# jhhung/kISS

Hardware: AMD Instinct MI355X
Metric: bases/sec suffix_sort (chm13v2.0-size synthetic, k=256) (higher is better)
Workload: dtype u8; 1 GPU; suffix_sort genome-like synthetic n=3117292070 k=256 (stand-in for chm13v2.0.fa, BASELINE.json configs[1]); PARALLEL_SORTING; text resident in HBM, SA left in HBM; n=3117292070, k=256, seed=2, parallelism=single GPU, lms=905939973, lms_rounds=9, tied_after_round0_item_rounds=184319413, big_segment_item_rounds=72866550, workspace_bytes=80357006484, induce_passes=47

## Files before the change

### kiss_amd/csrc/api.hip

```cpp
#include "kiss_internal.hpp"
#include <cstdlib>
#include <chrono>
#include <mutex>
#include <cstring>
#include <new>

KTimer::KTimer(kiss_hip_ctx *c, int cls, uint64_t items) : ctx(c), idx(-1)
{
    if (!((ctx->profile_mask >> cls) & 1ull)) return;
    if (ctx->ev_used == ctx->ev_pool.size()) {
        kiss_hip_ctx::Ev e;
        if (hipEventCreate(&e.a) != hipSuccess || hipEventCreate(&e.b) != hipSuccess) return;
        e.cls = 0;
        ctx->ev_pool.push_back(e);
    }
    idx = (int)ctx->ev_used++;
    ctx->ev_pool[idx].cls = cls;
    ctx->stats.launches_kernel[cls]++;
    ctx->stats.items_kernel[cls] += items;
    (void)hipEventRecord(ctx->ev_pool[idx].a, ctx->stream);
}
KTimer::~KTimer()
{
    if (idx >= 0) (void)hipEventRecord(ctx->ev_pool[idx].b, ctx->stream);
// ... 35 lines not shown
    o.pair_keys = env_on("KISS_HIP_PAIR_KEYS");
    o.no_fc0_onepass = env_on("KISS_HIP_NO_FC0_ONEPASS");
    o.no_pair_records = env_on("KISS_HIP_NO_PAIR_RECORDS");
    o.no_small_fused = env_on("KISS_HIP_NO_SMALL_FUSED");
    o.no_class_bytes = env_on("KISS_HIP_NO_CLASS_BYTES");
    o.no_pivot_ctx = env_on("KISS_HIP_NO_PIVOT_CTX");
    o.no_taint = env_on("KISS_HIP_NO_TAINT");
    o.isa_direct = env_on("KISS_HIP_ISA_DIRECT");
    o.no_onesweep = env_on("KISS_HIP_NO_ONESWEEP");
    o.rx_one_tile = env_on("KISS_HIP_RX_ONE_TILE");
    o.merge_lms = env_on("KISS_HIP_MERGE_LMS");
    o.no_small_alphabet = env_on("KISS_HIP_NO_SMALL_ALPHABET");
    o.induce_one_pass = env_on("KISS_HIP_INDUCE_ONE_PASS");
    o.verify = env_on("KISS_HIP_VERIFY");
    o.no_prefault = env_on("KISS_HIP_NO_PREFAULT");
    o.doubling_h0 = (uint32_t)env_u64("KISS_HIP_DOUBLING_H0", 0);
    o.tcap0 = env_u64("KISS_HIP_TCAP0", 0);
    o.pivot_slots = (int)env_u64("KISS_HIP_PIVOT_SLOTS", 3);
    o.small_seg = (uint32_t)env_u64("KISS_HIP_SMALL_SEG", 0);
    o.near_merge_min = (uint32_t)env_u64("KISS_HIP_NEAR_MERGE_MIN", 4096);
    o.induce_small_max = (uint32_t)env_u64("KISS_HIP_INDUCE_SMALL_MAX", 0);
    o.collapse_cap = (uint32_t)env_u64("KISS_HIP_COLLAPSE_CAP", 0);
    o.collapse_n = env_u64("KISS_HIP_COLLAPSE_N", 0);
    o.fm_heavy = (uint32_t)env_u64("KISS_HIP_FM_HEAVY", 0);
    o.fm_light = (uint32_t)env_u64("KISS_HIP_FM_LIGHT", 0);
    o.fm_mm_wave = env_on("KISS_HIP_FM_MM_WAVE");
    o.fm_mm_budget = env_u64("KISS_HIP_FM_MM_BUDGET", 0);
    o.fm8_group = env_on("KISS_HIP_FM8_GROUP");
    o.isa_direct_max = env_u64("KISS_HIP_ISA_DIRECT_MAX", 0);
    o.lx_sync_points = (unsigned)env_u64("KISS_HIP_LX_SYNC_POINTS", 0);
    o.tie_trace = (unsigned)env_u64("KISS_HIP_TIE_TRACE", 0);
    o.poison = (uint32_t)env_u64("KISS_HIP_POISON", 0);
    if (const char *e = getenv("KISS_HIP_DUMP_PIVOT")) snprintf(o.dump_pivot, sizeof o.dump_pivot, "%s", e);
    ctx->opts = o;
}
static std::mutex &kiss_launch_mutex()
{
    static std::mutex m;
    return m;
}
static bool kiss_lock_launches()
{
    static const bool on = getenv("KISS_HIP_LOCK_LAUNCHES") != nullptr;
    return on;
}
bool kiss_sync_launches()
// ... 98 lines not shown
    ctx->t_cap = 0;
    ctx->flags_cap = 0;
}

void free_lms_side(kiss_hip_ctx *ctx)
{
    free_tied(ctx);
    void **ptrs[] = {(void **)&ctx->lms_pos, (void **)&ctx->keyA, (void **)&ctx->keyB, (void **)&ctx->posA,
                     (void **)&ctx->posB, (void **)&ctx->lms_sorted_far, (void **)&ctx->lms_ctx_far,
                     (void **)&ctx->lmsP, (void **)&ctx->lmsC, (void **)&ctx->tile_hist, (void **)&ctx->scan_tmp,
                     (void **)&ctx->rx_desc, (void **)&ctx->rx_ghist, (void **)&ctx->fc_desc};
    for (void **p : ptrs)
        if (*p) {
            (void)hipFree(*p);
            *p = nullptr;
        }
    ctx->ws_bytes -= ctx->lms_bytes;
    ctx->lms_bytes = 0;
}

void free_all(kiss_hip_ctx *ctx)
{
    free_lms_side(ctx);
    void *ptrs[] = {ctx->pk, ctx->tile_gp, ctx->tile_cnt, ctx->cl_part, ctx->d_counts, ctx->CTX, ctx->CLS, ctx->ind_counts, ctx->ind_desc,
                    ctx->d_small, ctx->near_idx, ctx->near_fin, ctx->near_pos, ctx->near_tmp, ctx->near_tmp2, ctx->pairs1, ctx->pairs2, ctx->rx_ctl, ctx->refine_heads, ctx->ga_codes};
    for (void *p : ptrs)
        if (p) (void)hipFree(p);
    for (void *p : ctx->fm_pool)
        if (p) (void)hipFree(p);
    for (hipEvent_t e : ctx->fm_mm_ev)
        if (e) (void)hipEventDestroy(e);
#ifdef KISS_HIP_HOOKS
    if (ctx->tie_dbg) (void)hipFree(ctx->tie_dbg);
#endif
    if (ctx->io_S) (void)hipFree(ctx->io_S);
    if (ctx->io_SA) (void)hipFree(ctx->io_SA);
    kiss_xfer_free(ctx);
    if (ctx->h_pinned) (void)hipHostFree(ctx->h_pinned);
    if (ctx->h_pub) (void)hipHostFree(ctx->h_pub);
    for (auto &e : ctx->ev_pool) {
        (void)hipEventDestroy(e.a);
        (void)hipEventDestroy(e.b);
    }
    if (ctx->own_stream) (void)hipStreamDestroy(ctx->own_stream);
}

int sort_dev_unlocked(kiss_hip_ctx *ctx, const uint8_t *d_S, uint64_t n, uint32_t k, int algo, uint32_t *d_SA, void *stream);
int sort_dev(kiss_hip_ctx *ctx, const uint8_t *d_S, uint64_t n, uint32_t k, int algo, uint32_t *d_SA, void *stream)
{
    if (!ctx) return KISS_HIP_E_INVALID;
    kiss_opts_refresh(ctx);
#ifdef KISS_NO_DEVICE_LOCK
    return sort_dev_unlocked(ctx, d_S, n, k, algo, d_SA, stream);
#endif
    if (ctx->opts.no_serialize) return sort_dev_unlocked(ctx, d_S, n, k, algo, d_SA, stream);
    std::lock_guard<std::mutex> lock(kiss_device_mutex(ctx->device));
// ... 129 lines not shown

int kiss_need_ctx_words(kiss_hip_ctx *ctx)
{
    if (ctx->CTX && ctx->CLS) return KISS_HIP_OK;
    if (!ctx->CTX) KTRY(dmalloc(ctx, &ctx->CTX, ctx->max_n + 2));
    if (!ctx->CLS) KTRY(dmalloc(ctx, &ctx->CLS, ctx->max_n + 2 + 64));
    return KISS_HIP_OK;
}

int kiss_lms_reserve(kiss_hip_ctx *ctx, uint64_t m_cap, uint64_t t_cap_wanted)
{
    const bool dbg = ctx->opts.debug;
    const auto t_begin = std::chrono::steady_clock::now();
    free_lms_side(ctx);
    if (dbg)
        fprintf(stderr, "[kiss_hip] lms_reserve(%llu): freed the old arrays in %.3f s\n", (unsigned long long)m_cap,
                std::chrono::duration<double>(std::chrono::steady_clock::now() - t_begin).count());
    const uint64_t before = ctx->ws_bytes;
    ctx->m_cap = m_cap;
    const uint64_t radix_tiles = m_cap / 2048 + 2;
    ctx->tile_hist_cap = 256 * radix_tiles + 256 * (radix_tiles / 64 + 2) + 8;
    uint64_t biggest_scan = m_cap;
    if (ctx->tile_hist_cap > biggest_scan) biggest_scan = ctx->tile_hist_cap;
    if (ctx->ind_tiles_cap > biggest_scan) biggest_scan = ctx->ind_tiles_cap;
    if (ctx->n_tiles_cap > biggest_scan) biggest_scan = ctx->n_tiles_cap;
    ctx->scan_tmp_cap = biggest_scan / 4096 + 16;
    int rc = KISS_HIP_OK;
    do {
#define ALLOC(p, cnt) if ((rc = dmalloc(ctx, &ctx->p, (cnt)))) break
        ALLOC(lms_pos, m_cap);
        ALLOC(keyA, m_cap);
        ALLOC(keyB, m_cap);
        ALLOC(posA, m_cap);
        ALLOC(posB, m_cap);
        ALLOC(lms_sorted_far, m_cap);
        ALLOC(lms_ctx_far, m_cap);
        ALLOC(lmsP, m_cap);
        ALLOC(lmsC, m_cap);
        ALLOC(tile_hist, ctx->tile_hist_cap);
        ALLOC(scan_tmp, ctx->scan_tmp_cap);
        ctx->rx_tiles_cap = m_cap / 16384 + 2;
        ALLOC(rx_desc, 256 * ctx->rx_tiles_cap);
        ALLOC(rx_ghist, 256 * 12);
        ctx->fc_desc_cap = 2 * (m_cap / 8192 + 4);
        ALLOC(fc_desc, ctx->fc_desc_cap);
#undef ALLOC
        if (hipMemset(ctx->rx_desc, 0, 256 * ctx->rx_tiles_cap * sizeof(uint64_t)) != hipSuccess) rc = KISS_HIP_E_HIP;
// ... 187 lines not shown
    ctx->device = device;
    ctx->max_n = max_n;
    ctx->m_cap0 = lms_capacity ? lms_capacity + 4096 : 0;
    kiss_opts_supported_from_env(ctx->opts);
    kiss_opts_refresh(ctx);
    int rc = KISS_HIP_OK;
    do {
        if (hipSetDevice(device) != hipSuccess || hipStreamCreate(&ctx->own_stream) != hipSuccess) {
            rc = KISS_HIP_E_HIP;
            break;
        }
        ctx->stream = ctx->own_stream;
        const uint64_t words = max_n / 32 + 8;
        ctx->pk_words = words;
        ctx->n_tiles_cap = words / 256 + 2;
        ctx->ind_tiles_cap = 4 * ((max_n + 1) / 1024 + 2) + 2;
#define ALLOC(p, cnt) if ((rc = dmalloc(ctx, &ctx->p, (cnt)))) break
        ALLOC(pk, words);
        ALLOC(tile_gp, ctx->n_tiles_cap);
        ALLOC(tile_cnt, ctx->n_tiles_cap);
        ALLOC(cl_part, (ctx->n_tiles_cap < 8192 ? ctx->n_tiles_cap : 8192) * (uint64_t)(KISS_R0_PASSES * 256));
        ALLOC(d_counts, 16);
        ALLOC(ind_counts, ctx->ind_tiles_cap);
        ctx->ind_desc_stride = (max_n + 1) / 1024 + 2;
        ALLOC(ind_desc, 4 * ctx->ind_desc_stride);
        if (hipMemset(ctx->ind_desc, 0, 4 * ctx->ind_desc_stride * sizeof(uint64_t)) != hipSuccess) {
            rc = KISS_HIP_E_HIP;
            break;
        }
        ALLOC(rx_ctl, 4);
        if (hipMemset(ctx->rx_ctl, 0, 4 * sizeof(uint32_t)) != hipSuccess) {
            rc = KISS_HIP_E_HIP;
            break;
        }

        ALLOC(d_small, 64);
#undef ALLOC
        if ((rc = kiss_lms_reserve(ctx, default_m_cap(ctx)))) break;
        void *hp = nullptr;
        if (hipHostMalloc(&hp, 64 * sizeof(uint32_t), hipHostMallocDefault) != hipSuccess) {
            rc = KISS_HIP_E_NOMEM;
            break;
        }
        ctx->h_pinned = reinterpret_cast<uint32_t *>(hp);
        void *pub = nullptr, *dpub = nullptr;
        if (hipHostMalloc(&pub, 32 * sizeof(uint32_t), hipHostMallocCoherent | hipHostMallocMapped) == hipSuccess) {
            std::memset(pub, 0, 32 * sizeof(uint32_t));
            if (hipHostGetDevicePointer(&dpub, pub, 0) == hipSuccess) {
                ctx->h_pub = reinterpret_cast<uint32_t *>(pub);
                ctx->d_pub = reinterpret_cast<uint32_t *>(dpub);
            } else {
                (void)hipHostFree(pub);
// ... 251 lines not shown
```

### kiss_amd/csrc/induce.hip

```cpp
#include "kiss_internal.hpp"
#include <cstdio>
#include <cstdlib>

namespace {

constexpr int IN_THREADS = 256;
#ifndef KISS_IN_ITEMS
#define KISS_IN_ITEMS 8
#endif
constexpr int IN_ITEMS = KISS_IN_ITEMS;
constexpr int IN_WAVES = IN_THREADS / 64;
constexpr int IN_TILE = IN_THREADS * IN_ITEMS;
constexpr int SM_THREADS = 1024;
constexpr uint64_t SMALL_MAX = 8192;

__device__ __forceinline__ uint32_t child_ctx(uint32_t parent)
{
    return (KISS_CTX_WORD(parent) >> 2) | (parent & KISS_CTX_TAINT);
}

__device__ __forceinline__ uint32_t cls_byte(uint32_t c)
{
    return (c & 3u) | ((c & 0x7FFFFFFEu) == 0u ? 4u : 0u);
}
// ... 76 lines not shown
    uint32_t c = srcC[idx];
    if (KISS_CTX_WORD(c) <= KISS_EMPTY_CTX) {
        const uint32_t v = srcP[idx];
        if (v == 0) return 4u;
        c = kiss_load_ctx(pk, v) | (c & KISS_CTX_TAINT);
        srcC[idx] = c;
        if (srcK) srcK[idx] = (uint8_t)cls_byte(c);
    }
    const uint32_t pc = c & 3u;
    return ((emitmask >> pc) & 1u) ? pc : 4u;
}

__device__ __forceinline__ uint32_t wave_scan_add(uint32_t x)
{
    x += (uint32_t)__builtin_amdgcn_update_dpp(0, (int)x, 0x111, 0xf, 0xf, true);
    x += (uint32_t)__builtin_amdgcn_update_dpp(0, (int)x, 0x112, 0xf, 0xf, true);
    x += (uint32_t)__builtin_amdgcn_update_dpp(0, (int)x, 0x114, 0xf, 0xf, true);
    x += (uint32_t)__builtin_amdgcn_update_dpp(0, (int)x, 0x118, 0xf, 0xf, true);
    x += (uint32_t)__builtin_amdgcn_update_dpp(0, (int)x, 0x142, 0xa, 0xf, true);
    x += (uint32_t)__builtin_amdgcn_update_dpp(0, (int)x, 0x143, 0xc, 0xf, true);
    return x;
}

template <bool REMAP>
__global__ __launch_bounds__(IN_THREADS) void k_induce_count(const uint64_t *__restrict__ pk, const uint32_t *srcP,
                                                            uint32_t *srcC, int64_t beg, uint64_t N, int dir,
                                                            uint32_t emitmask, uint32_t *__restrict__ counts,
                                                            uint64_t tiles, LmsRemap rm, uint8_t *srcK)
{
    if (blockIdx.x == 0 && threadIdx.x == 4) counts[4 * tiles] = 0;
    const uint64_t tile = (uint64_t)blockIdx.x * IN_WAVES + (threadIdx.x >> 6);
    if (tile >= tiles) return;
    struct __attribute__((packed, aligned(4))) U4 {
        uint32_t v[4];
    };
    constexpr int STEPS = IN_TILE / 256;
    const uint32_t lane = lane_id();
    const uint64_t t0 = tile * IN_TILE;
    uint64_t acc = 0;
    int64_t shift = 0;
    bool block = t0 + IN_TILE <= N;
    if (REMAP && block) {
        const uint32_t b0 = remap_below_wave(rm, (uint64_t)beg + t0);
        block = b0 == remap_below_wave(rm, (uint64_t)beg + t0 + IN_TILE);
        shift = (int64_t)b0;
    }
    bool counted = false;
    if (!REMAP && srcK != nullptr && block) {
        const int64_t lo_index = dir > 0 ? beg + (int64_t)t0 : beg - (int64_t)(t0 + IN_TILE - 1);
        const uint8_t *const A = srcK + lo_index;
        const uint32_t mis = (uint32_t)(reinterpret_cast<uintptr_t>(A) & 15u);
        const uint4 *const ap = reinterpret_cast<const uint4 *>(A - mis);
        static_assert(IN_TILE == 2048, "64 lanes x 2 x 16 bytes");
        uint32_t w[12];
        {
            const uint4 q0 = ap[lane], q1 = ap[64 + lane];
            w[0] = q0.x, w[1] = q0.y, w[2] = q0.z, w[3] = q0.w;
            w[4] = q1.x, w[5] = q1.y, w[6] = q1.z, w[7] = q1.w;
            w[8] = w[9] = w[10] = w[11] = 0x08080808u;
        }
        if (mis != 0 && lane == 0) {
            const uint4 q2 = ap[128];
            const uint32_t tail[4] = {q2.x, q2.y, q2.z, q2.w};
#pragma unroll
            for (int i = 0; i < 4; i++) {
                const int nb = (int)mis - 4 * i;
                const uint32_t lowmask = nb >= 4 ? 0xFFFFFFFFu : (nb <= 0 ? 0u : ~(0xFFFFFFFFu << (8 * nb)));
                w[i] = (w[i] & ~lowmask) | (0x08080808u & lowmask);
                w[8 + i] = (tail[i] & lowmask) | (0x08080808u & ~lowmask);
            }
        }
        uint32_t any = 0;
#pragma unroll
        for (int i = 0; i < 12; i++) any |= w[i];
        if (__ballot((any & 0x04040404u) != 0u) == 0ull) {
            uint32_t cnt8 = 0;
#pragma unroll
            for (int i = 0; i < 12; i++) {
#pragma unroll
                for (int e = 0; e < 4; e++) {
                    const uint32_t b = (w[i] >> (8 * e)) & 0xFFu;
                    const uint32_t pc = b & 3u;
                    cnt8 += ((emitmask >> pc) & ~(b >> 3) & 1u) << (pc << 3);
                }
            }
            acc = (uint64_t)((cnt8 & 0xFFu) | ((cnt8 & 0xFF00u) << 8)) | ((uint64_t)(((cnt8 >> 16) & 0xFFu) | ((cnt8 >> 8) & 0xFF0000u)) << 32);
            counted = true;
        }
    }
    if (counted) {
    } else if (block) {
        U4 t[STEPS];
        int64_t p0[STEPS];
        uint32_t least = 0xFFFFFFFFu;
#pragma unroll
        for (int q = 0; q < STEPS; q++) {
            const uint64_t i0 = t0 + (uint64_t)q * 256 + 4 * lane;
            p0[q] = (dir > 0 ? beg + (int64_t)i0 : beg - (int64_t)(i0 + 3)) - shift;
            t[q] = *reinterpret_cast<const U4 *>(srcC + p0[q]);
        }
#pragma unroll
        for (int q = 0; q < STEPS; q++)
#pragma unroll
            for (int e = 0; e < 4; e++) least = min(least, t[q].v[e] & 0x7FFFFFFEu);
        uint32_t cnt8 = 0;
        if (__ballot(least == 0u) == 0ull) {
#pragma unroll
            for (int q = 0; q < STEPS; q++) {
#pragma unroll
                for (int e = 0; e < 4; e++) {
                    const uint32_t pc = t[q].v[e] & 3u;
                    cnt8 += ((emitmask >> pc) & 1u) << (pc << 3);
                }
            }
        } else {
#pragma unroll
            for (int q = 0; q < STEPS; q++) {
#pragma unroll
                for (int e = 0; e < 4; e++) {
                    const uint32_t c = t[q].v[e];
                    uint32_t cls;
                    if (KISS_CTX_WORD(c) <= KISS_EMPTY_CTX) cls = item_class_only<false>(pk, srcP, srcC, p0[q] + e, emitmask, rm, REMAP ? nullptr : srcK);
                    else {
                        const uint32_t pc = c & 3u;
                        cls = ((emitmask >> pc) & 1u) ? pc : 4u;
                    }
                    cnt8 += (cls < 4u ? 1u : 0u) << ((cls & 3u) << 3);
                }
            }
        }
        static_assert(IN_TILE / 64 <= 255, "8-bit counters per lane");
        acc = (uint64_t)((cnt8 & 0xFFu) | ((cnt8 & 0xFF00u) << 8)) | ((uint64_t)(((cnt8 >> 16) & 0xFFu) | ((cnt8 >> 8) & 0xFF0000u)) << 32);
    } else {
        for (uint64_t i = t0 + lane; i < N && i < t0 + IN_TILE; i += 64) {
            const uint32_t cls = item_class_only<REMAP>(pk, srcP, srcC, beg + (int64_t)dir * (int64_t)i, emitmask, rm, REMAP ? nullptr : srcK);
            acc += cls < 4u ? 1ull << (16 * cls) : 0ull;
        }
    }
    const uint32_t slo = (uint32_t)__builtin_amdgcn_readlane((int)wave_scan_add((uint32_t)acc), 63);
    const uint32_t shi = (uint32_t)__builtin_amdgcn_readlane((int)wave_scan_add((uint32_t)(acc >> 32)), 63);
    acc = ((uint64_t)shi << 32) | slo;
    if (lane < 4) counts[(uint64_t)lane * tiles + tile] = (uint32_t)(acc >> (16 * lane)) & 0xFFFFu;
}

struct DstPos {
    int64_t p[4];
};

template <bool REMAP, int DIR>
__global__ __launch_bounds__(IN_THREADS) void k_induce_scatter(const uint64_t *__restrict__ pk, const uint32_t *srcP,
                                                              uint32_t *srcC, int64_t beg, uint64_t N,
                                                              uint32_t emitmask, const uint32_t *__restrict__ ex,
                                                              uint64_t tiles, DstPos dst, uint32_t *SA, uint32_t *CTX,
                                                              uint32_t *__restrict__ totals, LmsRemap rm,
                                                              uint8_t *CLS,
                                                              uint8_t *srcK)
{
    static_assert(IN_ITEMS == 8 && IN_WAVES == 4, "8-bit counters per thread, 4-bit ranks of a thread's items in one word");
    static_assert(!REMAP || DIR > 0, "the LMS list is read left to right only");
    __shared__ uint32_t wtot[IN_WAVES][2];
    __shared__ __attribute__((aligned(16))) uint32_t stP[IN_TILE];
    __shared__ __attribute__((aligned(16))) uint32_t stC[IN_TILE];
    if (blockIdx.x == 0 && threadIdx.x < 4) totals[threadIdx.x] = ex[(uint64_t)(threadIdx.x + 1) * tiles] - ex[(uint64_t)threadIdx.x * tiles];
    const int wave = threadIdx.x >> 6;
    struct __attribute__((packed, aligned(4))) U4 {
        uint32_t v[4];
    };
    const uint64_t i0 = (uint64_t)blockIdx.x * IN_TILE + (uint64_t)threadIdx.x * IN_ITEMS;
    uint32_t vv[IN_ITEMS], cc[IN_ITEMS];
    uint32_t okm = 0;
    uint32_t loc = 0;
    uint32_t cnt8 = 0;
    auto take = [&](int e, uint32_t pc, uint32_t ok) {
        const uint32_t sh = pc << 3;
        loc |= ((cnt8 >> sh) & 15u) << (4 * e);
        cnt8 += ok << sh;
        okm |= ok << e;
    };
    int64_t shift = 0;
    bool block = i0 + IN_ITEMS <= N;
    if (REMAP) {
        const uint64_t tj = (uint64_t)beg + (uint64_t)blockIdx.x * IN_TILE;
        const uint32_t t0 = remap_below_wave(rm, tj), t1 = remap_below_wave(rm, tj + IN_TILE);
        if (t0 == t1) shift = (int64_t)t0;
        else if (block) {
            const uint32_t b0 = remap_below(rm, (uint64_t)beg + i0);
// ... 69 lines not shown
        tlo += a;
        thi += b;
        if (w < wave) {
            olo += a;
            ohi += b;
        }
    }
    const uint32_t c1 = tlo & 0xFFFFu, c2 = c1 + (tlo >> 16), c3 = c2 + (thi & 0xFFFFu), total = c3 + (thi >> 16);
    const uint32_t blo = (c1 << 16) + olo + (inlo - mylo), bhi = (c2 | (c3 << 16)) + ohi + (inhi - myhi);
#pragma unroll
    for (int e = 0; e < IN_ITEMS; e++) {
        if ((okm >> e) & 1u) {
            const uint32_t pc = cc[e] & 3u;
            const uint32_t base = __builtin_amdgcn_perm(bhi, blo, 0x0c0c0100u + pc * 0x0202u);
            const uint32_t li = base + ((loc >> (4 * e)) & 15u);
            stP[li] = vv[e] - 1u;
            stC[li] = child_ctx(cc[e]);
        }
    }
    __syncthreads();
    int64_t db[4];
    {
        const uint32_t cs[4] = {0u, c1, c2, c3};
#pragma unroll
        for (int k = 0; k < 4; k++) {
            const uint32_t toff = ex[(uint64_t)k * tiles + blockIdx.x] - ex[(uint64_t)k * tiles];
            db[k] = dst.p[k] + (int64_t)DIR * ((int64_t)toff - (int64_t)cs[k]);
        }
    }
    for (uint32_t l0 = threadIdx.x * 4u; l0 < total; l0 += IN_THREADS * 4u) {
        const uint32_t cls = (l0 >= c1 ? 1u : 0u) + (l0 >= c2 ? 1u : 0u) + (l0 >= c3 ? 1u : 0u);
        const uint32_t cend = cls == 0 ? c1 : (cls == 1 ? c2 : (cls == 2 ? c3 : total));
        if (l0 + 4u <= cend) {
            const int64_t dbk = cls == 0 ? db[0] : (cls == 1 ? db[1] : (cls == 2 ? db[2] : db[3]));
            const int64_t d0 = dbk + (int64_t)DIR * (int64_t)l0;
            const uint4 sp = *reinterpret_cast<const uint4 *>(stP + l0), sc = *reinterpret_cast<const uint4 *>(stC + l0);
            U4 wp, wc;
            if (DIR > 0) {
                wp.v[0] = sp.x, wp.v[1] = sp.y, wp.v[2] = sp.z, wp.v[3] = sp.w;
                wc.v[0] = sc.x, wc.v[1] = sc.y, wc.v[2] = sc.z, wc.v[3] = sc.w;
            } else {
                wp.v[0] = sp.w, wp.v[1] = sp.z, wp.v[2] = sp.y, wp.v[3] = sp.x;
                wc.v[0] = sc.w, wc.v[1] = sc.z, wc.v[2] = sc.y, wc.v[3] = sc.x;
            }
            const int64_t lo = DIR > 0 ? d0 : d0 - 3;
            *reinterpret_cast<U4 *>(SA + lo) = wp;
            *reinterpret_cast<U4 *>(CTX + lo) = wc;
            if (CLS) {
                struct __attribute__((packed, aligned(1))) B4 {
                    uint32_t v;
                };
                reinterpret_cast<B4 *>(CLS + lo)->v =
                    cls_byte(wc.v[0]) | (cls_byte(wc.v[1]) << 8) | (cls_byte(wc.v[2]) << 16) | (cls_byte(wc.v[3]) << 24);
            }
        } else {
            for (uint32_t li = l0; li < l0 + 4u && li < total; li++) {
                const uint32_t c2_ = (li >= c1 ? 1u : 0u) + (li >= c2 ? 1u : 0u) + (li >= c3 ? 1u : 0u);
                const int64_t dbk = c2_ == 0 ? db[0] : (c2_ == 1 ? db[1] : (c2_ == 2 ? db[2] : db[3]));
                const int64_t d = dbk + (int64_t)DIR * (int64_t)li;
                SA[d] = stP[li];
                CTX[d] = stC[li];
                if (CLS) CLS[d] = (uint8_t)cls_byte(stC[li]);
            }
        }
    }
}

constexpr uint32_t IN_SPIN_LIMIT = 1u << 22;
static_assert(IN_WAVES == 4, "wave c of a partition tile walks class c");

__device__ __forceinline__ uint32_t in_lookback(uint64_t *__restrict__ d, uint32_t tile, uint32_t mine, uint64_t tag,
                                                uint32_t *__restrict__ err)
{
    const uint32_t lane = lane_id();
    constexpr uint64_t TAGMASK = 0x3FFFFFFFull << 32;
    if (tile == 0) {
        if (lane == 0) __hip_atomic_store(&d[0], (2ull << 62) | tag | mine, __ATOMIC_RELAXED, __HIP_MEMORY_SCOPE_AGENT);
        return 0u;
    }
    if (lane == 0) __hip_atomic_store(&d[tile], (1ull << 62) | tag | mine, __ATOMIC_RELAXED, __HIP_MEMORY_SCOPE_AGENT);
    uint32_t excl = 0, spins = 0;
    int64_t base = (int64_t)tile;
    for (;;) {
        const int64_t t = base - 1 - (int64_t)lane;
        uint64_t v = t >= 0 ? __hip_atomic_load(&d[t], __ATOMIC_RELAXED, __HIP_MEMORY_SCOPE_AGENT) : ((2ull << 62) | tag);
        if ((v & TAGMASK) != tag) v = 0;
        const uint32_t st = (uint32_t)(v >> 62);
        const uint64_t incl = __ballot(st == 2u), ready = __ballot(st != 0u);
        const uint32_t first = incl ? (uint32_t)__builtin_ctzll(incl) : 64u;
        const uint64_t need = first >= 63u ? ~0ull : ((2ull << first) - 1ull);
// ... 167 lines not shown
            U4 wp, wc;
#pragma unroll
            for (int e = 0; e < 4; e++) {
                const int a = dir > 0 ? e : 3 - e;
                wp.v[a] = stP[l0 + e];
                wc.v[a] = stC[l0 + e];
            }
            const int64_t lo = dir > 0 ? d0 : d0 - 3;
            *reinterpret_cast<U4 *>(SA + lo) = wp;
            *reinterpret_cast<U4 *>(CTX + lo) = wc;
        } else {
            for (uint32_t li = l0; li < l0 + 4u && li < total; li++) {
                const uint32_t c2 = li < coff[1] ? 0u : (li < coff[2] ? 1u : (li < coff[3] ? 2u : 3u));
                const uint32_t toff = s_excl[c2];
                const uint32_t cstart = c2 == 0 ? coff[0] : (c2 == 1 ? coff[1] : (c2 == 2 ? coff[2] : coff[3]));
                const int64_t dp = c2 == 0 ? dst.p[0] : (c2 == 1 ? dst.p[1] : (c2 == 2 ? dst.p[2] : dst.p[3]));
                const int64_t d = dp + (int64_t)dir * (int64_t)((uint64_t)toff + (li - cstart));
                SA[d] = stP[li];
                CTX[d] = stC[li];
            }
        }
    }
}

template <bool REMAP>
__global__ __launch_bounds__(SM_THREADS) void k_induce_small(const uint64_t *__restrict__ pk, const uint32_t *srcP0,
                                                            uint32_t *srcC0, int64_t beg0, uint64_t N0, int dir,
                                                            uint32_t emitmask, int selfclass, DstPos dst, uint32_t *SA,
                                                            uint32_t *CTX, uint32_t *out, LmsRemap rm, uint8_t *CLS)
{
    __shared__ int64_t heads[4];
    __shared__ uint32_t wtot[SM_THREADS / 64][4];
    __shared__ uint32_t chunk_tot[4];
    __shared__ uint32_t round_self;
    if (threadIdx.x < 4) heads[threadIdx.x] = dst.p[threadIdx.x];
    if (threadIdx.x == 0) round_self = 0;
    __syncthreads();

    const uint32_t *srcP = srcP0;
    uint32_t *srcC = srcC0;
    int64_t beg = beg0;
    uint64_t N = N0;
    uint32_t rounds = 0;
    const int wave = threadIdx.x >> 6;

    while (N > 0) {
// ... 27 lines not shown
            }
            if (threadIdx.x < 4) {
                uint32_t t = 0;
                for (int w = 0; w < SM_THREADS / 64; w++) t += wtot[w][threadIdx.x];
                chunk_tot[threadIdx.x] = t;
            }
            __syncthreads();
            if (threadIdx.x < 4) heads[threadIdx.x] += (int64_t)dir * (int64_t)chunk_tot[threadIdx.x];
            if (threadIdx.x == 0 && selfclass >= 0) round_self += chunk_tot[selfclass];
            __syncthreads();
        }
        if (selfclass < 0) break;
        uint64_t nextN = round_self;
        __syncthreads();
        if (threadIdx.x == 0) round_self = 0;
        srcP = SA;
        srcC = CTX;
        beg = self_head_at_start;
        N = nextN;
        __syncthreads();
    }
    if (threadIdx.x < 4) out[threadIdx.x] = (uint32_t)((heads[threadIdx.x] - dst.p[threadIdx.x]) * (int64_t)dir);
    if (threadIdx.x == 0) out[4] = rounds;
}

struct Sweep {
    kiss_hip_ctx *ctx;
    uint32_t *SA;
    int dir;
    int64_t pos[4];
};

int run_pass(Sweep &sw, const uint32_t *srcP, uint32_t *srcC, int64_t beg, uint64_t N, uint32_t emitmask,
             int selfclass, uint64_t tot[4], bool *chain_done, const LmsRemap *remap = nullptr)
{
    kiss_hip_ctx *ctx = sw.ctx;
    const LmsRemap rm = remap ? *remap : LmsRemap{nullptr, nullptr, 0u};
    if (remap && (sw.dir < 0 || selfclass >= 0)) return KINTERNAL();
    for (int c = 0; c < 4; c++) tot[c] = 0;
    *chain_done = false;
    if (N == 0 || emitmask == 0) {
        *chain_done = true;
        return KISS_HIP_OK;
    }
    DstPos dp;
    for (int c = 0; c < 4; c++) dp.p[c] = sw.pos[c];
    ctx->stats.induce_passes++;
    uint8_t *const srcK = (srcC == ctx->CTX && ctx->CLS && !ctx->opts.no_class_bytes && !ctx->opts.induce_one_pass) ? ctx->CLS : nullptr;
    const uint64_t small_max = ctx->opts.induce_small_max >= 64 && ctx->opts.induce_small_max <= (1u << 20) ? ctx->opts.induce_small_max
                                                                                                           : (uint64_t)SMALL_MAX;
    if (N <= small_max) {
        {
            KTimer t(ctx, KISS_HIP_K_INDUCE_SMALL, N);
            if (remap)
                hipLaunchKernelGGL(k_induce_small<true>, dim3(1), dim3(SM_THREADS), 0, ctx->stream, ctx->pk, srcP, srcC, beg, N,
                                   sw.dir, emitmask, selfclass, dp, sw.SA, ctx->CTX, ctx->d_small, rm, ctx->CLS);
            else
                hipLaunchKernelGGL(k_induce_small<false>, dim3(1), dim3(SM_THREADS), 0, ctx->stream, ctx->pk, srcP, srcC, beg, N,
                                   sw.dir, emitmask, selfclass, dp, sw.SA, ctx->CTX, ctx->d_small, rm, ctx->CLS);
            KCHECK(hipGetLastError());
        }
        KTRY(kiss_readback(ctx, ctx->d_small, 5));
        for (int c = 0; c < 4; c++) tot[c] = ctx->h_pinned[c];
        *chain_done = true;
    } else {
        const uint64_t tiles = div_up(N, IN_TILE);
        if (4 * tiles + 1 > ctx->ind_tiles_cap) return KINTERNAL();
#ifdef KISS_HIP_HOOKS
        if (ctx->opts.induce_one_pass && ctx->ind_desc && tiles <= ctx->ind_desc_stride && tiles < (1ull << 31)) {
            KTimer t(ctx, KISS_HIP_K_INDUCE_SCATTER, N);
            ctx->ind_epoch++;
            if (remap)
                hipLaunchKernelGGL(k_induce_onepass<true>, dim3((unsigned)tiles), dim3(IN_THREADS), 0, ctx->stream, ctx->pk, srcP,
                                   srcC, beg, N, sw.dir, emitmask, tiles, dp, sw.SA, ctx->CTX, ctx->d_small, rm, ctx->ind_desc,
                                   ctx->ind_desc_stride, ctx->rx_ctl, ctx->ind_ticket_base, ctx->ind_epoch);
            else
                hipLaunchKernelGGL(k_induce_onepass<false>, dim3((unsigned)tiles), dim3(IN_THREADS), 0, ctx->stream, ctx->pk, srcP,
                                   srcC, beg, N, sw.dir, emitmask, tiles, dp, sw.SA, ctx->CTX, ctx->d_small, rm, ctx->ind_desc,
                                   ctx->ind_desc_stride, ctx->rx_ctl, ctx->ind_ticket_base, ctx->ind_epoch);
            KCHECK(hipGetLastError());
            ctx->ind_ticket_base += (uint32_t)tiles;
        } else
#endif
        {
        {
            KTimer t(ctx, KISS_HIP_K_INDUCE_COUNT, N);
            if (remap)
                hipLaunchKernelGGL(k_induce_count<true>, dim3((unsigned)div_up(tiles, IN_WAVES)), dim3(IN_THREADS), 0, ctx->stream,
                                   ctx->pk, srcP, srcC, beg, N, sw.dir, emitmask, ctx->ind_counts, tiles, rm, srcK);
            else
                hipLaunchKernelGGL(k_induce_count<false>, dim3((unsigned)div_up(tiles, IN_WAVES)), dim3(IN_THREADS), 0, ctx->stream,
                                   ctx->pk, srcP, srcC, beg, N, sw.dir, emitmask, ctx->ind_counts, tiles, rm, srcK);
            KCHECK(hipGetLastError());
        }
        KTRY(kiss_scan_u32(ctx, ctx->ind_counts, ctx->ind_counts, 4 * tiles + 1));
        {
            KTimer t(ctx, KISS_HIP_K_INDUCE_SCATTER, N);
            if (remap)
                hipLaunchKernelGGL((k_induce_scatter<true, 1>), dim3((unsigned)tiles), dim3(IN_THREADS), 0, ctx->stream, ctx->pk, srcP,
                                   srcC, beg, N, emitmask, ctx->ind_counts, tiles, dp, sw.SA, ctx->CTX, ctx->d_small, rm, ctx->CLS, srcK);
            else if (sw.dir > 0)
                hipLaunchKernelGGL((k_induce_scatter<false, 1>), dim3((unsigned)tiles), dim3(IN_THREADS), 0, ctx->stream, ctx->pk, srcP,
                                   srcC, beg, N, emitmask, ctx->ind_counts, tiles, dp, sw.SA, ctx->CTX, ctx->d_small, rm, ctx->CLS, srcK);
            else
                hipLaunchKernelGGL((k_induce_scatter<false, -1>), dim3((unsigned)tiles), dim3(IN_THREADS), 0, ctx->stream, ctx->pk, srcP,
                                   srcC, beg, N, emitmask, ctx->ind_counts, tiles, dp, sw.SA, ctx->CTX, ctx->d_small, rm, ctx->CLS, srcK);
            KCHECK(hipGetLastError());
        }
        }
        KTRY(kiss_readback(ctx, ctx->d_small, 4));
        for (int c = 0; c < 4; c++) tot[c] = ctx->h_pinned[c];
    }
    if (ctx->opts.debug)
        fprintf(stderr, "[kiss_hip] pass dir=%d beg=%lld N=%llu mask=%x self=%d -> %llu,%llu,%llu,%llu\n", sw.dir, (long long)beg,
                (unsigned long long)N, emitmask, selfclass, (unsigned long long)tot[0], (unsigned long long)tot[1],
                (unsigned long long)tot[2], (unsigned long long)tot[3]);
    for (int c = 0; c < 4; c++) sw.pos[c] += (int64_t)sw.dir * (int64_t)tot[c];
    return KISS_HIP_OK;
}

constexpr uint64_t COLLAPSE_N = 1ull << 18;
constexpr uint32_t COLLAPSE_RCAP = 65535;
constexpr uint32_t COLLAPSE_RCAP_WIDE = (1u << 22) - 1;
constexpr int CH_THREADS = 256;

constexpr uint32_t RUN_SERIAL = 1024;

__device__ __forceinline__ uint32_t run_before(const uint64_t *__restrict__ pk, uint64_t v, uint32_t c, uint32_t cap,
                                               bool valid)
// ... 390 lines not shown
```

### kiss_amd/csrc/kiss_internal.hpp

```cpp
#pragma once
#include <hip/hip_runtime.h>
#include <stdint.h>
#include <stddef.h>
#include <mutex>
#include <vector>
#include "../../include/kiss_hip.h"

struct KissOpts {
    bool debug = false;
    int xfer_threads = 0;
    int prefault_threads = 0;
    bool sync_readback = false;
    bool no_lms_exact = false;
    bool heads_by_compare = false;
    bool no_early_out = false;
    bool no_pivot_rounds = false;
    bool pivot_from_round2 = false;
    bool pair_keys = false;
    bool no_fc0_onepass = false;
    bool no_pair_records = false;
    bool no_small_fused = false;
    bool no_class_bytes = false;
    bool no_pivot_ctx = false;
    bool no_taint = false;
    bool isa_direct = false;
    bool no_onesweep = false;
    bool rx_one_tile = false;
    bool merge_lms = false;
    bool no_small_alphabet = false;
    bool induce_one_pass = false;
    bool verify = false;
    bool no_prefault = false;
    bool no_serialize = false;
    bool lock_launches = false;
    bool sync_launches = false;
    uint32_t doubling_h0 = 0;
    uint64_t tcap0 = 0;
    int pivot_slots = 3;
    uint32_t small_seg = 0;
    uint32_t near_merge_min = 4096;
    uint32_t induce_small_max = 0;
    uint32_t collapse_cap = 0;
    uint64_t collapse_n = 0;
    uint32_t fm_heavy = 0, fm_light = 0;
    bool fm_mm_wave = false;
    bool fm8_group = false;
    uint64_t fm_mm_budget = 0;
    uint64_t isa_direct_max = 0;
    unsigned lx_sync_points = 0;
    unsigned tie_trace = 0;
    uint32_t poison = 0;
    char dump_pivot[256] = {0};
};
struct kiss_hip_ctx;
#ifdef KISS_HIP_HOOKS
void kiss_opts_refresh(kiss_hip_ctx *ctx);
struct KissLaunchGuard {
    bool held;
    KissLaunchGuard();
    ~KissLaunchGuard();
};
bool kiss_sync_launches();
#define KISS_ARG4_(a, b, c, d, ...) d
#ifdef hipLaunchKernelGGL
#undef hipLaunchKernelGGL
#define hipLaunchKernelGGL(kernelName, ...)                                                                            \
// ... 68 lines not shown
    uint32_t *segstartA = nullptr, *segstartB = nullptr;
    uint64_t *bkeyA = nullptr, *bkeyB = nullptr;
    uint32_t *bposA = nullptr, *bposB = nullptr, *bsegA = nullptr, *bsegB = nullptr, *bslot = nullptr;
    uint64_t *flags = nullptr;
    uint32_t *lms_sorted_far = nullptr;
    uint32_t *lms_ctx_far = nullptr;
    uint32_t *lmsP = nullptr;
    uint32_t *lmsC = nullptr;
    uint32_t *tile_hist = nullptr;
    uint64_t tile_hist_cap = 0;
    uint64_t *rx_desc = nullptr;
    uint32_t *rx_ghist = nullptr, *rx_ctl = nullptr;
    uint64_t rx_ghist_count = 0;
    uint64_t rx_tiles_cap = 0, rx_epoch = 0;
    uint64_t *fc_desc = nullptr;
    uint64_t fc_desc_cap = 0;
    uint32_t rx_ticket_base = 0;
    uint64_t *scan_tmp = nullptr;
    uint64_t scan_tmp_cap = 0;
    uint32_t *CTX = nullptr;
    bool ctx_words_valid = false;
    uint32_t *ind_counts = nullptr;
    uint64_t ind_tiles_cap = 0;
    uint64_t *ind_desc = nullptr;
    uint64_t ind_desc_stride = 0, ind_epoch = 0;
    uint32_t ind_ticket_base = 0;
    uint32_t *d_small = nullptr;
    uint32_t *h_pinned = nullptr;
    uint32_t *h_pub = nullptr;
    uint32_t *d_pub = nullptr;
    uint32_t pub_seq = 0;
    int pub_mode = -1;
    uint64_t *pairs1 = nullptr, *pairs2 = nullptr;
    uint64_t pairs_cap = 0;
    void *fm_pool[36] = {};
    uint64_t fm_pool_cap[36] = {};
    hipEvent_t fm_mm_ev[6] = {};
    uint32_t *near_idx = nullptr, *near_fin = nullptr, *near_pos = nullptr, *near_tmp = nullptr, *near_tmp2 = nullptr;
    uint64_t near_cap = 0;
    uint8_t *ga_codes = nullptr;
    uint64_t ga_codes_cap = 0;
    uint8_t *refine_heads = nullptr;
    uint8_t *hfar = nullptr, *hmerged = nullptr;
    uint32_t h_depth = 0;
    bool lms_merged = false;
    int near_form = 0;
    const uint32_t *near_sorted = nullptr;
    const uint32_t *rm_fin = nullptr, *rm_pos = nullptr;
    uint32_t rm_E = 0;
// ... 142 lines not shown
```

Before: 47.26 billion bases/s.

## Group induce count tiles per wave and scan only per-group totals

The induce count kernel now has each wave walk a group of consecutive tiles. It writes a local running prefix per tile and a single total per group, so the global scan covers only the group totals. When class bytes are present it loads four tiles at once with wide vector loads, which raises memory-level parallelism, and it reuses the remap boundary between tiles. The scatter kernel combines the group offset with the in-group tile offset. The one-pass descriptor path and its allocation are moved under the hooks build flag. The cost is a smaller grid and one extra indexed read in the scatter kernel.

```diff
diff --git a/kiss_amd/csrc/api.hip b/kiss_amd/csrc/api.hip
--- a/kiss_amd/csrc/api.hip
+++ b/kiss_amd/csrc/api.hip
@@ -81,6 +81,7 @@
     o.induce_small_max = (uint32_t)env_u64("KISS_HIP_INDUCE_SMALL_MAX", 0);
     o.collapse_cap = (uint32_t)env_u64("KISS_HIP_COLLAPSE_CAP", 0);
     o.collapse_n = env_u64("KISS_HIP_COLLAPSE_N", 0);
+    o.induce_group_tiles = (uint32_t)env_u64("KISS_HIP_INDUCE_GROUP_TILES", 0);
     o.fm_heavy = (uint32_t)env_u64("KISS_HIP_FM_HEAVY", 0);
     o.fm_light = (uint32_t)env_u64("KISS_HIP_FM_LIGHT", 0);
     o.fm_mm_wave = env_on("KISS_HIP_FM_MM_WAVE");
@@ -225,7 +226,7 @@
 void free_all(kiss_hip_ctx *ctx)
 {
     free_lms_side(ctx);
-    void *ptrs[] = {ctx->pk, ctx->tile_gp, ctx->tile_cnt, ctx->cl_part, ctx->d_counts, ctx->CTX, ctx->CLS, ctx->ind_counts, ctx->ind_desc,
+    void *ptrs[] = {ctx->pk, ctx->tile_gp, ctx->tile_cnt, ctx->cl_part, ctx->d_counts, ctx->CTX, ctx->CLS, ctx->ind_counts, ctx->ind_gtot,
                     ctx->d_small, ctx->near_idx, ctx->near_fin, ctx->near_pos, ctx->near_tmp, ctx->near_tmp2, ctx->pairs1, ctx->pairs2, ctx->rx_ctl, ctx->refine_heads, ctx->ga_codes};
     for (void *p : ptrs)
         if (p) (void)hipFree(p);
@@ -235,6 +236,7 @@
         if (e) (void)hipEventDestroy(e);
 #ifdef KISS_HIP_HOOKS
     if (ctx->tie_dbg) (void)hipFree(ctx->tie_dbg);
+    if (ctx->ind_desc) (void)hipFree(ctx->ind_desc);
 #endif
     if (ctx->io_S) (void)hipFree(ctx->io_S);
     if (ctx->io_SA) (void)hipFree(ctx->io_SA);
@@ -410,7 +412,7 @@
     ctx->tile_hist_cap = 256 * radix_tiles + 256 * (radix_tiles / 64 + 2) + 8;
     uint64_t biggest_scan = m_cap;
     if (ctx->tile_hist_cap > biggest_scan) biggest_scan = ctx->tile_hist_cap;
-    if (ctx->ind_tiles_cap > biggest_scan) biggest_scan = ctx->ind_tiles_cap;
+    if (ctx->ind_groups_cap > biggest_scan) biggest_scan = ctx->ind_groups_cap;
     if (ctx->n_tiles_cap > biggest_scan) biggest_scan = ctx->n_tiles_cap;
     ctx->scan_tmp_cap = biggest_scan / 4096 + 16;
     int rc = KISS_HIP_OK;
@@ -644,12 +646,16 @@
         ALLOC(cl_part, (ctx->n_tiles_cap < 8192 ? ctx->n_tiles_cap : 8192) * (uint64_t)(KISS_R0_PASSES * 256));
         ALLOC(d_counts, 16);
         ALLOC(ind_counts, ctx->ind_tiles_cap);
+        ctx->ind_groups_cap = ctx->ind_tiles_cap;
+        ALLOC(ind_gtot, ctx->ind_groups_cap);
+#ifdef KISS_HIP_HOOKS
         ctx->ind_desc_stride = (max_n + 1) / 1024 + 2;
         ALLOC(ind_desc, 4 * ctx->ind_desc_stride);
         if (hipMemset(ctx->ind_desc, 0, 4 * ctx->ind_desc_stride * sizeof(uint64_t)) != hipSuccess) {
             rc = KISS_HIP_E_HIP;
             break;
         }
+#endif
         ALLOC(rx_ctl, 4);
         if (hipMemset(ctx->rx_ctl, 0, 4 * sizeof(uint32_t)) != hipSuccess) {
             rc = KISS_HIP_E_HIP;
diff --git a/kiss_amd/csrc/induce.hip b/kiss_amd/csrc/induce.hip
--- a/kiss_amd/csrc/induce.hip
+++ b/kiss_amd/csrc/induce.hip
@@ -122,82 +122,86 @@
     return x;
 }
 
+struct __attribute__((packed, aligned(4))) CntU4 {
+    uint32_t v[4];
+};
+
+__device__ __forceinline__ uint64_t cnt8_spread(uint32_t cnt8)
+{
+    return (uint64_t)((cnt8 & 0xFFu) | ((cnt8 & 0xFF00u) << 8)) | ((uint64_t)(((cnt8 >> 16) & 0xFFu) | ((cnt8 >> 8) & 0xFF0000u)) << 32);
+}
+
+static_assert(IN_TILE == 2048, "64 lanes x 2 x 16 bytes");
+template <int NT>
+__device__ __forceinline__ void cls_tiles_load(const uint8_t *A, uint32_t lane, uint32_t w[NT][8], uint32_t last[4])
+{
+    const uint32_t mis = (uint32_t)(reinterpret_cast<uintptr_t>(A) & 15u);
+    const uint4 *const ap = reinterpret_cast<const uint4 *>(A - mis);
+#pragma unroll
+    for (int b = 0; b < NT; b++) {
+        const uint4 q0 = ap[128 * b + lane], q1 = ap[128 * b + 64 + lane];
+        w[b][0] = q0.x, w[b][1] = q0.y, w[b][2] = q0.z, w[b][3] = q0.w;
+        w[b][4] = q1.x, w[b][5] = q1.y, w[b][6] = q1.z, w[b][7] = q1.w;
+    }
+    uint4 q2 = make_uint4(0u, 0u, 0u, 0u);
+    if (mis != 0 && lane == 0) q2 = ap[128 * NT];
+    last[0] = q2.x, last[1] = q2.y, last[2] = q2.z, last[3] = q2.w;
+}
+
+__device__ __forceinline__ void cls_lowmask(const uint8_t *A, uint32_t lane, uint32_t lowmask[4])
+{
+    const uint32_t mis = lane == 0 ? (uint32_t)(reinterpret_cast<uintptr_t>(A) & 15u) : 0u;
+#pragma unroll
+    for (int i = 0; i < 4; i++) {
+        const int nb = (int)mis - 4 * i;
+        lowmask[i] = nb >= 4 ? 0xFFFFFFFFu : (nb <= 0 ? 0u : ~(0xFFFFFFFFu << (8 * nb)));
+    }
+}
+
+__device__ __forceinline__ bool cls_tile_count(const uint32_t w[8], const uint32_t next[4], const uint32_t lowmask[4],
+                                               uint32_t emitmask, uint64_t *acc)
+{
+    uint32_t x[12];
+#pragma unroll
+    for (int i = 0; i < 4; i++) {
+        x[i] = (w[i] & ~lowmask[i]) | (0x08080808u & lowmask[i]);
+        x[4 + i] = w[4 + i];
+        x[8 + i] = (next[i] & lowmask[i]) | (0x08080808u & ~lowmask[i]);
+    }
+    uint32_t any = 0;
+#pragma unroll
+    for (int i = 0; i < 12; i++) any |= x[i];
+    if (__ballot((any & 0x04040404u) != 0u) != 0ull) return false;
+    uint32_t cnt8 = 0;
+#pragma unroll
+    for (int i = 0; i < 12; i++) {
+#pragma unroll
+        for (int e = 0; e < 4; e++) {
+            const uint32_t b = (x[i] >> (8 * e)) & 0xFFu;
+            const uint32_t pc = b & 3u;
+            cnt8 += ((emitmask >> pc) & ~(b >> 3) & 1u) << (pc << 3);
+        }
+    }
+    *acc = cnt8_spread(cnt8);
+    return true;
+}
+
 template <bool REMAP>
-__global__ __launch_bounds__(IN_THREADS) void k_induce_count(const uint64_t *__restrict__ pk, const uint32_t *srcP,
-                                                            uint32_t *srcC, int64_t beg, uint64_t N, int dir,
-                                                            uint32_t emitmask, uint32_t *__restrict__ counts,
-                                                            uint64_t tiles, LmsRemap rm, uint8_t *srcK)
-{
-    if (blockIdx.x == 0 && threadIdx.x == 4) counts[4 * tiles] = 0;
-    const uint64_t tile = (uint64_t)blockIdx.x * IN_WAVES + (threadIdx.x >> 6);
-    if (tile >= tiles) return;
-    struct __attribute__((packed, aligned(4))) U4 {
-        uint32_t v[4];
-    };
+__device__ __forceinline__ uint64_t words_tile_count(const uint64_t *__restrict__ pk, const uint32_t *srcP, uint32_t *srcC,
+                                                     int64_t beg, uint64_t N, int dir, uint32_t emitmask, uint64_t t0,
+                                                     bool block, int64_t shift, const LmsRemap &rm, uint8_t *srcK)
+{
     constexpr int STEPS = IN_TILE / 256;
     const uint32_t lane = lane_id();
-    const uint64_t t0 = tile * IN_TILE;
-    uint64_t acc = 0;
-    int64_t shift = 0;
-    bool block = t0 + IN_TILE <= N;
-    if (REMAP && block) {
-        const uint32_t b0 = remap_below_wave(rm, (uint64_t)beg + t0);
-        block = b0 == remap_below_wave(rm, (uint64_t)beg + t0 + IN_TILE);
-        shift = (int64_t)b0;
-    }
-    bool counted = false;
-    if (!REMAP && srcK != nullptr && block) {
-        const int64_t lo_index = dir > 0 ? beg + (int64_t)t0 : beg - (int64_t)(t0 + IN_TILE - 1);
-        const uint8_t *const A = srcK + lo_index;
-        const uint32_t mis = (uint32_t)(reinterpret_cast<uintptr_t>(A) & 15u);
-        const uint4 *const ap = reinterpret_cast<const uint4 *>(A - mis);
-        static_assert(IN_TILE == 2048, "64 lanes x 2 x 16 bytes");
-        uint32_t w[12];
-        {
-            const uint4 q0 = ap[lane], q1 = ap[64 + lane];
-            w[0] = q0.x, w[1] = q0.y, w[2] = q0.z, w[3] = q0.w;
-            w[4] = q1.x, w[5] = q1.y, w[6] = q1.z, w[7] = q1.w;
-            w[8] = w[9] = w[10] = w[11] = 0x08080808u;
-        }
-        if (mis != 0 && lane == 0) {
-            const uint4 q2 = ap[128];
-            const uint32_t tail[4] = {q2.x, q2.y, q2.z, q2.w};
-#pragma unroll
-            for (int i = 0; i < 4; i++) {
-                const int nb = (int)mis - 4 * i;
-                const uint32_t lowmask = nb >= 4 ? 0xFFFFFFFFu : (nb <= 0 ? 0u : ~(0xFFFFFFFFu << (8 * nb)));
-                w[i] = (w[i] & ~lowmask) | (0x08080808u & lowmask);
-                w[8 + i] = (tail[i] & lowmask) | (0x08080808u & ~lowmask);
-            }
-        }
-        uint32_t any = 0;
-#pragma unroll
-        for (int i = 0; i < 12; i++) any |= w[i];
-        if (__ballot((any & 0x04040404u) != 0u) == 0ull) {
-            uint32_t cnt8 = 0;
-#pragma unroll
-            for (int i = 0; i < 12; i++) {
-#pragma unroll
-                for (int e = 0; e < 4; e++) {
-                    const uint32_t b = (w[i] >> (8 * e)) & 0xFFu;
-                    const uint32_t pc = b & 3u;
-                    cnt8 += ((emitmask >> pc) & ~(b >> 3) & 1u) << (pc << 3);
-                }
-            }
-            acc = (uint64_t)((cnt8 & 0xFFu) | ((cnt8 & 0xFF00u) << 8)) | ((uint64_t)(((cnt8 >> 16) & 0xFFu) | ((cnt8 >> 8) & 0xFF0000u)) << 32);
-            counted = true;
-        }
-    }
-    if (counted) {
-    } else if (block) {
-        U4 t[STEPS];
+    if (block) {
+        CntU4 t[STEPS];
         int64_t p0[STEPS];
         uint32_t least = 0xFFFFFFFFu;
 #pragma unroll
         for (int q = 0; q < STEPS; q++) {
             const uint64_t i0 = t0 + (uint64_t)q * 256 + 4 * lane;
             p0[q] = (dir > 0 ? beg + (int64_t)i0 : beg - (int64_t)(i0 + 3)) - shift;
-            t[q] = *reinterpret_cast<const U4 *>(srcC + p0[q]);
+            t[q] = *reinterpret_cast<const CntU4 *>(srcC + p0[q]);
         }
 #pragma unroll
         for (int q = 0; q < STEPS; q++)
@@ -230,17 +234,85 @@
             }
         }
         static_assert(IN_TILE / 64 <= 255, "8-bit counters per lane");
-        acc = (uint64_t)((cnt8 & 0xFFu) | ((cnt8 & 0xFF00u) << 8)) | ((uint64_t)(((cnt8 >> 16) & 0xFFu) | ((cnt8 >> 8) & 0xFF0000u)) << 32);
-    } else {
-        for (uint64_t i = t0 + lane; i < N && i < t0 + IN_TILE; i += 64) {
-            const uint32_t cls = item_class_only<REMAP>(pk, srcP, srcC, beg + (int64_t)dir * (int64_t)i, emitmask, rm, REMAP ? nullptr : srcK);
-            acc += cls < 4u ? 1ull << (16 * cls) : 0ull;
-        }
-    }
-    const uint32_t slo = (uint32_t)__builtin_amdgcn_readlane((int)wave_scan_add((uint32_t)acc), 63);
-    const uint32_t shi = (uint32_t)__builtin_amdgcn_readlane((int)wave_scan_add((uint32_t)(acc >> 32)), 63);
-    acc = ((uint64_t)shi << 32) | slo;
-    if (lane < 4) counts[(uint64_t)lane * tiles + tile] = (uint32_t)(acc >> (16 * lane)) & 0xFFFFu;
+        return cnt8_spread(cnt8);
+    }
+    uint64_t acc = 0;
+    for (uint64_t i = t0 + lane; i < N && i < t0 + IN_TILE; i += 64) {
+        const uint32_t cls = item_class_only<REMAP>(pk, srcP, srcC, beg + (int64_t)dir * (int64_t)i, emitmask, rm, REMAP ? nullptr : srcK);
+        acc += cls < 4u ? 1ull << (16 * cls) : 0ull;
+    }
+    return acc;
+}
+
+constexpr int IN_CNT_AHEAD = 4;
+template <bool REMAP>
+__global__ __launch_bounds__(IN_THREADS, 4) void k_induce_count(const uint64_t *__restrict__ pk, const uint32_t *srcP,
+                                                               uint32_t *srcC, int64_t beg, uint64_t N, int dir,
+                                                               uint32_t emitmask, uint32_t *__restrict__ counts,
+                                                               uint32_t *__restrict__ gtot, uint64_t tiles, uint32_t G,
+                                                               uint32_t groups, LmsRemap rm, uint8_t *srcK)
+{
+    if (blockIdx.x == 0 && threadIdx.x == 4) gtot[4 * (uint64_t)groups] = 0;
+    const uint32_t grp = blockIdx.x * IN_WAVES + (uint32_t)__builtin_amdgcn_readfirstlane((int)(threadIdx.x >> 6));
+    if (grp >= groups) return;
+    const uint32_t lane = lane_id();
+    const uint64_t tbeg = (uint64_t)grp * G;
+    const uint64_t tend = tbeg + G < tiles ? tbeg + G : tiles;
+    uint32_t run = 0;
+    auto tile_done = [&](uint64_t tile, uint64_t acc) {
+        const uint32_t slo = (uint32_t)__builtin_amdgcn_readlane((int)wave_scan_add((uint32_t)acc), 63);
+        const uint32_t shi = (uint32_t)__builtin_amdgcn_readlane((int)wave_scan_add((uint32_t)(acc >> 32)), 63);
+        const uint64_t tot = ((uint64_t)shi << 32) | slo;
+        if (lane < 4) {
+            counts[(uint64_t)lane * tiles + tile] = run;
+            run += (uint32_t)(tot >> (16 * lane)) & 0xFFFFu;
+        }
+    };
+    uint32_t rb = 0;
+    bool have_rb = false;
+    const bool bytes = !REMAP && srcK != nullptr;
+    auto tile_bytes = [&](uint64_t t0, int nt) { return srcK + (dir > 0 ? beg + (int64_t)t0 : beg - (int64_t)(t0 + (uint64_t)nt * IN_TILE - 1)); };
+    uint32_t lowmask[4] = {0u, 0u, 0u, 0u};
+    if (bytes) cls_lowmask(tile_bytes(0, 1), lane, lowmask);
+    uint64_t tile = tbeg;
+    while (tile < tend) {
+        const uint64_t t0 = tile * IN_TILE;
+        if (bytes && tile + IN_CNT_AHEAD <= tend && t0 + (uint64_t)IN_CNT_AHEAD * IN_TILE <= N) {
+            uint32_t w[IN_CNT_AHEAD][8], last[4];
+            uint64_t acc[IN_CNT_AHEAD];
+            cls_tiles_load<IN_CNT_AHEAD>(tile_bytes(t0, IN_CNT_AHEAD), lane, w, last);
+            bool ok = true;
+#pragma unroll
+            for (int a = 0; a < IN_CNT_AHEAD; a++)
+                ok &= cls_tile_count(w[a], a + 1 < IN_CNT_AHEAD ? w[(a + 1) % IN_CNT_AHEAD] : last, lowmask, emitmask, &acc[a]);
+            if (ok) {
+#pragma unroll
+                for (int b = 0; b < IN_CNT_AHEAD; b++) tile_done(tile + b, dir > 0 ? acc[b] : acc[IN_CNT_AHEAD - 1 - b]);
+                tile += IN_CNT_AHEAD;
+                continue;
+            }
+        }
+        int64_t shift = 0;
+        bool block = t0 + IN_TILE <= N;
+        if (REMAP && block) {
+            const uint32_t b0 = have_rb ? rb : remap_below_wave(rm, (uint64_t)beg + t0);
+            rb = remap_below_wave(rm, (uint64_t)beg + t0 + IN_TILE);
+            have_rb = true;
+            block = b0 == rb;
+            shift = (int64_t)b0;
+        }
+        uint64_t acc = 0;
+        bool counted = false;
+        if (bytes && block) {
+            uint32_t w[1][8], last[4];
+            cls_tiles_load<1>(tile_bytes(t0, 1), lane, w, last);
+            counted = cls_tile_count(w[0], last, lowmask, emitmask, &acc);
+        }
+        if (!counted) acc = words_tile_count<REMAP>(pk, srcP, srcC, beg, N, dir, emitmask, t0, block, shift, rm, srcK);
+        tile_done(tile, acc);
+        tile++;
+    }
+    if (lane < 4) gtot[(uint64_t)lane * groups + grp] = run;
 }
 
 struct DstPos {
@@ -251,7 +323,8 @@
 __global__ __launch_bounds__(IN_THREADS) void k_induce_scatter(const uint64_t *__restrict__ pk, const uint32_t *srcP,
                                                               uint32_t *srcC, int64_t beg, uint64_t N,
                                                               uint32_t emitmask, const uint32_t *__restrict__ ex,
-                                                              uint64_t tiles, DstPos dst, uint32_t *SA, uint32_t *CTX,
+                                                              const uint32_t *__restrict__ gex, uint64_t tiles, uint32_t G,
+                                                              uint32_t groups, DstPos dst, uint32_t *SA, uint32_t *CTX,
                                                               uint32_t *__restrict__ totals, LmsRemap rm,
                                                               uint8_t *CLS,
                                                               uint8_t *srcK)
@@ -261,7 +334,7 @@
     __shared__ uint32_t wtot[IN_WAVES][2];
     __shared__ __attribute__((aligned(16))) uint32_t stP[IN_TILE];
     __shared__ __attribute__((aligned(16))) uint32_t stC[IN_TILE];
-    if (blockIdx.x == 0 && threadIdx.x < 4) totals[threadIdx.x] = ex[(uint64_t)(threadIdx.x + 1) * tiles] - ex[(uint64_t)threadIdx.x * tiles];
+    if (blockIdx.x == 0 && threadIdx.x < 4) totals[threadIdx.x] = gex[(threadIdx.x + 1) * groups] - gex[threadIdx.x * groups];
     const int wave = threadIdx.x >> 6;
     struct __attribute__((packed, aligned(4))) U4 {
         uint32_t v[4];
@@ -377,9 +450,10 @@
     int64_t db[4];
     {
         const uint32_t cs[4] = {0u, c1, c2, c3};
+        const uint32_t grp = blockIdx.x / G;
 #pragma unroll
         for (int k = 0; k < 4; k++) {
-            const uint32_t toff = ex[(uint64_t)k * tiles + blockIdx.x] - ex[(uint64_t)k * tiles];
+            const uint32_t toff = gex[k * groups + grp] - gex[k * groups] + ex[(uint64_t)k * tiles + blockIdx.x];
             db[k] = dst.p[k] + (int64_t)DIR * ((int64_t)toff - (int64_t)cs[k]);
         }
     }
@@ -421,6 +495,7 @@
     }
 }
 
+#ifdef KISS_HIP_HOOKS
 constexpr uint32_t IN_SPIN_LIMIT = 1u << 22;
 static_assert(IN_WAVES == 4, "wave c of a partition tile walks class c");
 
@@ -634,6 +709,7 @@
         }
     }
 }
+#endif
 
 template <bool REMAP>
 __global__ __launch_bounds__(SM_THREADS) void k_induce_small(const uint64_t *__restrict__ pk, const uint32_t *srcP0,
@@ -707,6 +783,12 @@
     }
     if (threadIdx.x < 4) out[threadIdx.x] = (uint32_t)((heads[threadIdx.x] - dst.p[threadIdx.x]) * (int64_t)dir);
     if (threadIdx.x == 0) out[4] = rounds;
+}
+
+uint32_t group_tiles(bool class_bytes, uint32_t forced)
+{
+    if (forced) return forced;
+    return class_bytes ? (uint32_t)IN_CNT_AHEAD : 1u;
 }
 
 struct Sweep {
@@ -751,6 +833,9 @@
     } else {
         const uint64_t tiles = div_up(N, IN_TILE);
         if (4 * tiles + 1 > ctx->ind_tiles_cap) return KINTERNAL();
+        const uint32_t G = group_tiles(srcK != nullptr && !remap, ctx->opts.induce_group_tiles);
+        const uint32_t groups = (uint32_t)div_up(tiles, G);
+        if (4 * (uint64_t)groups + 1 > ctx->ind_groups_cap) return KINTERNAL();
 #ifdef KISS_HIP_HOOKS
         if (ctx->opts.induce_one_pass && ctx->ind_desc && tiles <= ctx->ind_desc_stride && tiles < (1ull << 31)) {
             KTimer t(ctx, KISS_HIP_K_INDUCE_SCATTER, N);
@@ -771,25 +856,25 @@
         {
             KTimer t(ctx, KISS_HIP_K_INDUCE_COUNT, N);
             if (remap)
-                hipLaunchKernelGGL(k_induce_count<true>, dim3((unsigned)div_up(tiles, IN_WAVES)), dim3(IN_THREADS), 0, ctx->stream,
-                                   ctx->pk, srcP, srcC, beg, N, sw.dir, emitmask, ctx->ind_counts, tiles, rm, srcK);
+                hipLaunchKernelGGL(k_induce_count<true>, dim3((unsigned)div_up(groups, IN_WAVES)), dim3(IN_THREADS), 0, ctx->stream,
+                                   ctx->pk, srcP, srcC, beg, N, sw.dir, emitmask, ctx->ind_counts, ctx->ind_gtot, tiles, G, groups, rm, srcK);
             else
-                hipLaunchKernelGGL(k_induce_count<false>, dim3((unsigned)div_up(tiles, IN_WAVES)), dim3(IN_THREADS), 0, ctx->stream,
-                                   ctx->pk, srcP, srcC, beg, N, sw.dir, emitmask, ctx->ind_counts, tiles, rm, srcK);
+                hipLaunchKernelGGL(k_induce_count<false>, dim3((unsigned)div_up(groups, IN_WAVES)), dim3(IN_THREADS), 0, ctx->stream,
+                                   ctx->pk, srcP, srcC, beg, N, sw.dir, emitmask, ctx->ind_counts, ctx->ind_gtot, tiles, G, groups, rm, srcK);
             KCHECK(hipGetLastError());
         }
-        KTRY(kiss_scan_u32(ctx, ctx->ind_counts, ctx->ind_counts, 4 * tiles + 1));
+        KTRY(kiss_scan_u32(ctx, ctx->ind_gtot, ctx->ind_gtot, 4 * (uint64_t)groups + 1));
         {
             KTimer t(ctx, KISS_HIP_K_INDUCE_SCATTER, N);
             if (remap)
                 hipLaunchKernelGGL((k_induce_scatter<true, 1>), dim3((unsigned)tiles), dim3(IN_THREADS), 0, ctx->stream, ctx->pk, srcP,
-                                   srcC, beg, N, emitmask, ctx->ind_counts, tiles, dp, sw.SA, ctx->CTX, ctx->d_small, rm, ctx->CLS, srcK);
+                                   srcC, beg, N, emitmask, ctx->ind_counts, ctx->ind_gtot, tiles, G, groups, dp, sw.SA, ctx->CTX, ctx->d_small, rm, ctx->CLS, srcK);
             else if (sw.dir > 0)
                 hipLaunchKernelGGL((k_induce_scatter<false, 1>), dim3((unsigned)tiles), dim3(IN_THREADS), 0, ctx->stream, ctx->pk, srcP,
-                                   srcC, beg, N, emitmask, ctx->ind_counts, tiles, dp, sw.SA, ctx->CTX, ctx->d_small, rm, ctx->CLS, srcK);
+                                   srcC, beg, N, emitmask, ctx->ind_counts, ctx->ind_gtot, tiles, G, groups, dp, sw.SA, ctx->CTX, ctx->d_small, rm, ctx->CLS, srcK);
             else
                 hipLaunchKernelGGL((k_induce_scatter<false, -1>), dim3((unsigned)tiles), dim3(IN_THREADS), 0, ctx->stream, ctx->pk, srcP,
-                                   srcC, beg, N, emitmask, ctx->ind_counts, tiles, dp, sw.SA, ctx->CTX, ctx->d_small, rm, ctx->CLS, srcK);
+                                   srcC, beg, N, emitmask, ctx->ind_counts, ctx->ind_gtot, tiles, G, groups, dp, sw.SA, ctx->CTX, ctx->d_small, rm, ctx->CLS, srcK);
             KCHECK(hipGetLastError());
         }
         }
diff --git a/kiss_amd/csrc/kiss_internal.hpp b/kiss_amd/csrc/kiss_internal.hpp
--- a/kiss_amd/csrc/kiss_internal.hpp
+++ b/kiss_amd/csrc/kiss_internal.hpp
@@ -42,6 +42,7 @@
     uint32_t induce_small_max = 0;
     uint32_t collapse_cap = 0;
     uint64_t collapse_n = 0;
+    uint32_t induce_group_tiles = 0;
     uint32_t fm_heavy = 0, fm_light = 0;
     bool fm_mm_wave = false;
     bool fm8_group = false;
@@ -156,9 +157,13 @@
     bool ctx_words_valid = false;
     uint32_t *ind_counts = nullptr;
     uint64_t ind_tiles_cap = 0;
+    uint32_t *ind_gtot = nullptr;
+    uint64_t ind_groups_cap = 0;
+#ifdef KISS_HIP_HOOKS
     uint64_t *ind_desc = nullptr;
     uint64_t ind_desc_stride = 0, ind_epoch = 0;
     uint32_t ind_ticket_base = 0;
+#endif
     uint32_t *d_small = nullptr;
     uint32_t *h_pinned = nullptr;
     uint32_t *h_pub = nullptr;
```

Measured after the change: 47.16 billion bases/s. No clear change (-0.2%).
